# CPJKU/audio_sheet_retrieval

Measured on AMD Instinct MI355X. Metric: snippet-pairs/sec embedded+ranked (32-d CCA), higher is better.
Workload: dtype f32

## Files before the change

### audio_sheet_retrieval_amd/csrc/conv_wino4_kernels.hip

```cpp
#include <hip/hip_runtime.h>
#include <stdint.h>
#include <stdlib.h>
#include <algorithm>
#include <type_traits>
#include <vector>
#include "asr_kernels.h"
#include "repack_elems.inl"
#include "wino4_epilogue.h"

#ifndef ASR_WINO4_ABL
#define ASR_WINO4_ABL 0
#endif

namespace asr {

typedef float floatx4q __attribute__((ext_vector_type(4)));
typedef float float2q __attribute__((ext_vector_type(2)));

struct Wino4Args {
    const float *in, *wpk, *bnp;
    float *out;
    int N, H, W, OH, OW;
    int ty_img, tx_img;
    int coutp;
    int tiles;
    int total;
    double *stats;
    BnBwdFuse bf;
    int epi;
};

__device__ __forceinline__ float elu_fastq(float y) { return y > 0.0f ? y : __expf(y) - 1.0f; }

__device__ __forceinline__ floatx4q bn_elu4q(floatx4q x, float mean, float scale, float beta) {
    const floatx4q y = (x - floatx4q{mean, mean, mean, mean}) * floatx4q{scale, scale, scale, scale} +
                       floatx4q{beta, beta, beta, beta};
    return floatx4q{elu_fastq(y[0]), elu_fastq(y[1]), elu_fastq(y[2]), elu_fastq(y[3])};
}
typedef int int4q __attribute__((ext_vector_type(4)));
__device__ __forceinline__ void buffer_store_q(float v, unsigned voff, int4q rsrc, unsigned soff) {
    asm volatile("buffer_store_dword %0, %1, %2, %3 offen" ::"v"(v), "v"(voff), "s"(rsrc), "s"(soff) : "memory");
}

template <typename T> __device__ __forceinline__ T splatq(float c);
template <> __device__ __forceinline__ float2q splatq<float2q>(float c) { return float2q{c, c}; }
template <> __device__ __forceinline__ floatx4q splatq<floatx4q>(float c) { return floatx4q{c, c, c, c}; }
template <typename T> __device__ __forceinline__ T fmaq(float c, T x, T y) {
    return __builtin_elementwise_fma(splatq<T>(c), x, y);
}

template <typename T> __device__ __forceinline__ void in6(T &d0, T &d1, T &d2, T &d3, T &d4, T &d5) {
    const T r0 = fmaq(4.f, d0, fmaq(-5.f, d2, d4));
    const T t1 = fmaq(-4.f, d2, d4), t2 = fmaq(-4.f, d1, d3);
    const T t3 = d4 - d2, t4 = d3 - d1;
    const T r5 = fmaq(4.f, d1, fmaq(-5.f, d3, d5));
    d0 = r0; d1 = t1 + t2; d2 = t1 - t2; d3 = fmaq(2.f, t4, t3); d4 = fmaq(-2.f, t4, t3); d5 = r5;
}
template <typename T> __device__ __forceinline__ void out6(T m0, T m1, T m2, T m3, T m4, T m5, T &y0, T &y1, T &y2, T &y3) {
    const T s1 = m1 + m2, s2 = m1 - m2, s3 = m3 + m4, s4 = m3 - m4;
    y0 = (m0 + s1) + s3;
    y1 = fmaq(2.f, s4, s2);
    y2 = fmaq(4.f, s3, s1);
    y3 = fmaq(8.f, s4, s2) + m5;
}

template <int CIN, int COUT, bool POOL, int WAVES, bool RAW>
__global__ __launch_bounds__(64 * WAVES, 1) void conv3x3_wino4g(Wino4Args a) {
    constexpr int KS = CIN / 4, NB = CIN / 8, T = 64 * WAVES;
    constexpr int WS = 16;
    constexpr int WD = 6;
    constexpr int WQ = 72;
    static_assert(CIN % 8 == 0, "channel blocks of 8");
    extern __shared__ __align__(16) float w_lds[];
    const int tid = threadIdx.x, lane = tid & 63;
    const int wave = __builtin_amdgcn_readfirstlane(tid >> 6);
    const int nt0 = blockIdx.y;
    for (int i = tid; i < KS * 36 * 4 * 16; i += T) {
        const int row = i >> 4, nn = i & 15;
        const int gg = row & 3, kp = row >> 2, ks = kp / 36, p = kp - ks * 36;
        const int qq = (ks & 1) * 36 + p;
        w_lds[i] = a.wpk[((((size_t)(ks >> 1) * 18 + (qq >> 2)) * 4 + gg) * a.coutp + nt0 * 16 + nn) * 4 + (qq & 3)];
    }
    __syncthreads();

    const int m = lane & 15, g = lane >> 4, n = lane & 15;
    const float *w_lane = w_lds + g * WS + n;
    const int chn = nt0 * 16 + n;
    const bool ch_ok = chn < COUT;
    const float bmean = (!RAW && ch_ok) ? a.bnp[chn] : 0.f;
    const float bscale = (!RAW && ch_ok) ? a.bnp[a.coutp + chn] : 1.f;
    const float bbeta = (!RAW && ch_ok) ? a.bnp[2 * a.coutp + chn] : 0.f;
    const int per_img = a.ty_img * a.tx_img;

    for (int mt = blockIdx.x * WAVES + wave; mt < a.total; mt += gridDim.x * WAVES) {
        const int tnum = mt * 16 + m;
        const bool tvalid = tnum < a.tiles;
        const int tcl = min(tnum, a.tiles - 1);
        const int img = tcl / per_img;
        const int trest = tcl - img * per_img;
        const int tty = trest / a.tx_img, ttx = trest - tty * a.tx_img;
        const int py = 4 * tty, px = 4 * ttx;
        const float *ibase = a.in + (int64_t)img * a.H * a.W * CIN + 2 * g;
        int rowb[6], colb[6];
        unsigned oy_m = 0, ox_m = 0;
#pragma unroll
        for (int i = 0; i < 6; ++i) {
            const int y = py - 1 + i, x = px - 1 + i;
            oy_m |= (unsigned)(y >= 0 && y < a.H) << i;
            ox_m |= (unsigned)(x >= 0 && x < a.W) << i;
            rowb[i] = min(max(y, 0), a.H - 1) * a.W * CIN;
            colb[i] = min(max(x, 0), a.W - 1) * CIN;
        }
        if (!tvalid) oy_m = 0;
        const bool interior = __builtin_amdgcn_ballot_w64(oy_m != 0x3fu || ox_m != 0x3fu) == 0;
        unsigned my_off;
        int my_ext;
        if (POOL) {
            my_off = (((unsigned)img * a.OH + 2 * tty) * a.OW + 2 * ttx) * COUT;
            const int nr = min(2, a.OH - 2 * tty), nc = min(2, a.OW - 2 * ttx);
            my_ext = (tvalid && nr > 0 && nc > 0) ? (nr | (nc << 8)) : 0;
        } else {
            my_off = (((unsigned)img * a.H + py) * a.W + px) * COUT;
            const int nr = min(4, a.H - py), nc = min(4, a.W - px);
            my_ext = tvalid ? (nr | (nc << 8)) : 0;
        }

        floatx4q acc[36];
#pragma unroll
        for (int p = 0; p < 36; ++p) acc[p] = floatx4q{0.f, 0.f, 0.f, 0.f};

        float2q nxt[6][6];
#pragma unroll
        for (int i = 0; i < 6; ++i)
#pragma unroll
            for (int j = 0; j < 6; ++j) nxt[i][j] = *reinterpret_cast<const float2q *>(ibase + rowb[i] + colb[j]);
        float wpre[WD];
#pragma unroll
        for (int q = 0; q < WD; ++q) wpre[q] = w_lane[q * 4 * WS];
#pragma unroll 1
        for (int t = 0; t < NB; ++t) {
            float2q dp[6][6];
            if (interior) {
#pragma unroll
                for (int i = 0; i < 6; ++i)
#pragma unroll
                    for (int j = 0; j < 6; ++j) dp[i][j] = nxt[i][j];
            } else {
#pragma unroll
                for (int i = 0; i < 6; ++i)
#pragma unroll
                    for (int j = 0; j < 6; ++j)
                        dp[i][j] = (((oy_m >> i) & (ox_m >> j)) & 1u) ? nxt[i][j] : float2q{0.f, 0.f};
            }
            if (t + 1 < NB && !(ASR_WINO4_ABL & 2)) {
#pragma unroll
                for (int i = 0; i < 6; ++i)
#pragma unroll
                    for (int j = 0; j < 6; ++j)
                        nxt[i][j] = *reinterpret_cast<const float2q *>(ibase + rowb[i] + colb[j] + 8 * (t + 1));
            }
#pragma unroll
            for (int j = 0; j < 6; ++j) in6(dp[0][j], dp[1][j], dp[2][j], dp[3][j], dp[4][j], dp[5][j]);
#pragma unroll
            for (int i = 0; i < 6; ++i) in6(dp[i][0], dp[i][1], dp[i][2], dp[i][3], dp[i][4], dp[i][5]);
            const float *wk = w_lane + (2 * t) * (36 * 4 * WS);
            const float *wn = (t + 1 < NB) ? wk + 2 * 36 * 4 * WS : w_lane;
            float wv[WQ + WD];
#pragma unroll
            for (int q = 0; q < WD; ++q) wv[q] = wpre[q];
#pragma unroll
            for (int q0 = 0; q0 < WQ; q0 += 2) {
#pragma unroll
                for (int q = q0; q < q0 + 2; ++q)
                    wv[q + WD] = (q + WD < WQ) ? wk[(q + WD) * 4 * WS] : wn[(q + WD - WQ) * 4 * WS];
                __builtin_amdgcn_sched_barrier(0);
#pragma unroll
                for (int q = q0; q < q0 + 2; ++q) {
                    const int c = q / 36, p = q % 36;
                    acc[p] = __builtin_amdgcn_mfma_f32_16x16x4f32(dp[p / 6][p % 6][c], wv[q], acc[p], 0, 0, 0);
                }
                __builtin_amdgcn_sched_barrier(0);
            }
#pragma unroll
            for (int q = 0; q < WD; ++q) wpre[q] = wv[WQ + q];
        }

        unsigned eo[4];
        int ee[4];
#pragma unroll
        for (int r = 0; r < 4; ++r) {
            eo[r] = (unsigned)__shfl((int)my_off, 4 * g + r);
            ee[r] = __shfl(my_ext, 4 * g + r);
        }
        if (!ch_ok) continue;
        floatx4q tc[4][6];
#pragma unroll
        for (int nu = 0; nu < 6; ++nu)
            out6(acc[nu], acc[6 + nu], acc[12 + nu], acc[18 + nu], acc[24 + nu], acc[30 + nu], tc[0][nu], tc[1][nu], tc[2][nu],
                 tc[3][nu]);
        if (POOL) {
#pragma unroll
            for (int pr = 0; pr < 2; ++pr) {
                floatx4q ya[4], yb[4];
                out6(tc[2 * pr][0], tc[2 * pr][1], tc[2 * pr][2], tc[2 * pr][3], tc[2 * pr][4], tc[2 * pr][5], ya[0], ya[1],
                     ya[2], ya[3]);
                out6(tc[2 * pr + 1][0], tc[2 * pr + 1][1], tc[2 * pr + 1][2], tc[2 * pr + 1][3], tc[2 * pr + 1][4],
                     tc[2 * pr + 1][5], yb[0], yb[1], yb[2], yb[3]);
#pragma unroll
                for (int pc = 0; pc < 2; ++pc) {
#pragma unroll
                    for (int r = 0; r < 4; ++r) {
                        if (pr >= (ee[r] & 0xff) || pc >= (ee[r] >> 8)) continue;
                        const float v0 = ya[2 * pc][r], v1 = ya[2 * pc + 1][r], v2 = yb[2 * pc][r], v3 = yb[2 * pc + 1][r];
                        const float hi = fmaxf(fmaxf(v0, v1), fmaxf(v2, v3));
                        const float lo = fminf(fminf(v0, v1), fminf(v2, v3));
                        const float x = bscale >= 0.0f ? hi : lo;
                        a.out[(size_t)eo[r] + (size_t)(pr * a.OW + pc) * COUT + chn] =
                            elu_fastq((x - bmean) * bscale + bbeta);
                    }
                }
            }
        } else {
#pragma unroll
            for (int i = 0; i < 4; ++i) {
                floatx4q y[4];
                out6(tc[i][0], tc[i][1], tc[i][2], tc[i][3], tc[i][4], tc[i][5], y[0], y[1], y[2], y[3]);
#pragma unroll
                for (int j = 0; j < 4; ++j) {
#pragma unroll
                    for (int r = 0; r < 4; ++r) {
                        if (i >= (ee[r] & 0xff) || j >= (ee[r] >> 8)) continue;
                        const float v = RAW ? y[j][r] : elu_fastq((y[j][r] - bmean) * bscale + bbeta);
                        a.out[(size_t)eo[r] + (size_t)(i * a.W + j) * COUT + chn] = v;
                    }
                }
            }
        }
    }
}

template <int CIN, int COUT, bool POOL, int SLICE = COUT, int PW = 1, bool RAW = false>
__global__ __launch_bounds__(64 * (PW + (SLICE + 15) / 16), 1) void conv3x3_wino4s(Wino4Args a) {
    static_assert(!(RAW && POOL), "the raw form has no pooled epilogue");
    constexpr int NT = (SLICE + 15) / 16, NB = CIN / 8, KS = CIN / 4;
    static_assert(PW == 1 || PW == 2, "one or two producer waves");
    static_assert(PW + NT <= 4, "one wave per SIMD");
    static_assert(SLICE == COUT || (SLICE % 16 == 0 && COUT % SLICE == 0), "slices are whole n-tiles");
    constexpr int VB = 36 * 16 * 8;
    static_assert(CIN % 8 == 0, "channel blocks of 8");
    extern __shared__ __align__(16) float vbuf[];
    const int tid = threadIdx.x, lane = tid & 63;
    const int wave = __builtin_amdgcn_readfirstlane(tid >> 6);
    const bool producer = wave < PW;
    const int m = lane & 15, g = lane >> 4, n = lane & 15;
    const int per_img = a.ty_img * a.tx_img;

    int mt, mt_end, mt_stride;
    if ((gridDim.x & 7) == 0) {
        const int per_x = (a.total + 7) >> 3;
        const int r0 = (int)(blockIdx.x & 7) * per_x;
        mt_end = min(r0 + per_x, a.total);
        mt_stride = (int)(gridDim.x >> 3);
        mt = r0 + (int)(blockIdx.x >> 3);
    } else {
        mt_end = a.total; mt_stride = (int)gridDim.x; mt = (int)blockIdx.x;
    }
    if (mt >= mt_end) {
        if constexpr (RAW) {
            if (a.stats)
                for (int c = threadIdx.x; c < 2 * COUT; c += blockDim.x) a.stats[(size_t)blockIdx.x * 2 * COUT + c] = 0.0;
        }
        return;
    }

    auto tile_of = [&](int mtile, int &img, int &tty, int &ttx, bool &tvalid) {
        const int tnum = mtile * 16 + m;
        tvalid = tnum < a.tiles;
        const int tcl = min(tnum, a.tiles - 1);
        img = tcl / per_img;
        const int trest = tcl - img * per_img;
        tty = trest / a.tx_img;
        ttx = trest - tty * a.tx_img;
    };
    float *vlane = vbuf + (g * 32 + 2 * m);
#ifdef ASR_WINO4_OLD_V
    vlane = vbuf + (m * 8 + 2 * g);
#endif

    if (producer) {
        unsigned poff[6][6];
        unsigned oy_m = 0, ox_m = 0;
        auto setup = [&](int mtile) {
            int img, tty, ttx;
            bool tvalid;
            tile_of(mtile, img, tty, ttx, tvalid);
            const int py = 4 * tty, px = 4 * ttx;
            const unsigned ib = ((unsigned)img * a.H * a.W * CIN + 2 * g) * 4u;
            unsigned rowb[6], colb[6];
            oy_m = 0; ox_m = 0;
#pragma unroll
            for (int i = 0; i < 6; ++i) {
                const int y = py - 1 + i, x = px - 1 + i;
                oy_m |= (unsigned)(y >= 0 && y < a.H) << i;
                ox_m |= (unsigned)(x >= 0 && x < a.W) << i;
                rowb[i] = (unsigned)(min(max(y, 0), a.H - 1) * a.W * CIN) * 4u;
                colb[i] = (unsigned)(min(max(x, 0), a.W - 1) * CIN) * 4u;
            }
            if (!tvalid) oy_m = 0;
#pragma unroll
            for (int i = 0; i < 6; ++i)
#pragma unroll
                for (int j = 0; j < 6; ++j) poff[i][j] = ib + rowb[i] + colb[j];
        };
        float2q nxt[6][6];
        auto load = [&](int t) {
            const char *cb = reinterpret_cast<const char *>(a.in + 8 * t);
#pragma unroll
            for (int i = 0; i < 6; ++i)
#pragma unroll
                for (int j = 0; j < 6; ++j) nxt[i][j] = *reinterpret_cast<const float2q *>(cb + poff[i][j]);
        };
        const int n_mt = (mt_end - mt + mt_stride - 1) / mt_stride;
        const int n_steps = n_mt * NB;
        int passed = 0;
        int t = wave;
        while (t >= NB) { t -= NB; mt += mt_stride; }
        if (mt < mt_end) { setup(mt); load(t); }
        for (int step = wave; step < n_steps; step += PW) {
            float2q dp[6][6];
            const unsigned oy = oy_m, ox = ox_m;
            const bool interior = __builtin_amdgcn_ballot_w64(oy != 0x3fu || ox != 0x3fu) == 0;
            if (interior) {
#pragma unroll
                for (int i = 0; i < 6; ++i)
#pragma unroll
                    for (int j = 0; j < 6; ++j) dp[i][j] = nxt[i][j];
            } else {
#pragma unroll
                for (int i = 0; i < 6; ++i)
#pragma unroll
                    for (int j = 0; j < 6; ++j) dp[i][j] = (((oy >> i) & (ox >> j)) & 1u) ? nxt[i][j] : float2q{0.f, 0.f};
            }
            {
                int tn = t + PW, mtn = mt;
                while (tn >= NB) { tn -= NB; mtn += mt_stride; }
                if (!(ASR_WINO4_ABL & 2) && step + PW < n_steps) {
                    if (mtn != mt) setup(mtn);
                    load(tn);
                }
                t = tn; mt = mtn;
            }
            if (!(ASR_WINO4_ABL & 8)) {
#pragma unroll
            for (int j = 0; j < 6; ++j) in6(dp[0][j], dp[1][j], dp[2][j], dp[3][j], dp[4][j], dp[5][j]);
#pragma unroll
            for (int i = 0; i < 6; ++i) in6(dp[i][0], dp[i][1], dp[i][2], dp[i][3], dp[i][4], dp[i][5]);
            }
            while (passed < step) { __syncthreads(); ++passed; }
            float *vb = vlane + (step & 1) * VB;
            if (!(ASR_WINO4_ABL & 16)) {
#pragma unroll
            for (int p = 0; p < 36; ++p) *reinterpret_cast<float2q *>(vb + p * 128) = dp[p / 6][p % 6];
            } else {
#pragma unroll
            for (int p = 0; p < 36; ++p) asm volatile("" ::"v"(dp[p / 6][p % 6]));
            }
            __syncthreads();
            ++passed;
        }
        while (passed < n_steps + 1) { __syncthreads(); ++passed; }
        return;
    }

    const int nt = wave - PW;
    const int chn = (int)blockIdx.y * SLICE + nt * 16 + n;
    const bool ch_ok = chn < COUT;
    float bmean = (!RAW && ch_ok) ? a.bnp[chn] : 0.f;
    float bscale = (!RAW && ch_ok) ? a.bnp[a.coutp + chn] : 1.f;
    float bbeta = (!RAW && ch_ok) ? a.bnp[2 * a.coutp + chn] : 0.f;
    float bistd = 0.f;
    const bool bnb = ASR_BNB_FUSE_BUILD && RAW && a.stats && a.bf.z != nullptr;
    if (bnb && ch_ok) {
        bmean = a.bf.cst[chn]; bistd = a.bf.cst[COUT + chn];
        bscale = a.bf.cst[2 * COUT + chn]; bbeta = a.bf.cst[3 * COUT + chn];
    }
    double st1 = 0.0, st2 = 0.0;
    int4q orsrc;
    {
        const uint64_t obase = reinterpret_cast<uint64_t>(a.out);
        orsrc.x = (int)(uint32_t)obase;
        orsrc.y = (int)(uint32_t)(obase >> 32);
        orsrc.z = (int)((unsigned)a.N * a.OH * a.OW * COUT * 4u);
        orsrc.w = 0x00020000;
    }
    const unsigned wlane = ((unsigned)g * a.coutp + chn) * 16u;
    const float *wl = a.wpk;
    constexpr int wstep = 4 * ((COUT + 15) / 16 * 16);
    floatx4q bw[2][18];
#pragma unroll
    for (int j = 0; j < 18; ++j)
        bw[0][j] = *reinterpret_cast<const floatx4q *>(reinterpret_cast<const char *>(wl) + (size_t)j * (wstep * 16) + wlane);
    int step = 0;
    for (; mt < mt_end; mt += mt_stride) {
        unsigned my_off;
        int my_ext;
        {
            int img, tty, ttx;
            bool tvalid;
            tile_of(mt, img, tty, ttx, tvalid);
            if (POOL) my_off = (((unsigned)img * a.OH + 2 * tty) * a.OW + 2 * ttx) * COUT;
            else my_off = (((unsigned)img * a.H + 4 * tty) * a.W + 4 * ttx) * COUT;
            my_ext = wino4_extent(POOL, POOL ? a.OH : a.H, POOL ? a.OW : a.W, tty, ttx, tvalid);
        }
        int epi_mode = 0;
        if constexpr (!RAW) {
            if (a.epi)
                epi_mode = __builtin_amdgcn_ballot_w64(!wino4_rows_full(my_ext, POOL)) == 0 ? 1 : (wino4_general_form(POOL) ? 2 : 0);
        }
        unsigned voff[9];
#pragma unroll
        for (int k = 0; k < 9; ++k) {
            voff[k] = wlane + (unsigned)k * (2 * wstep * 16);
            asm volatile("" : "+v"(voff[k]));
        }
        floatx4q acc[36];
        auto reload = [&](const float *wn, auto set_c) {
            constexpr int SET = decltype(set_c)::value;
            if (ASR_WINO4_ABL & 4) return;
            const char *wnb = reinterpret_cast<const char *>(wn);
#pragma unroll
            for (int k = 0; k < 9; ++k) {
                unsigned vo = voff[k];
                asm volatile("" : "+v"(vo));
                bw[SET][2 * k] = *reinterpret_cast<const floatx4q *>(wnb + vo);
                bw[SET][2 * k + 1] = *reinterpret_cast<const floatx4q *>(wnb + (wstep * 16) + vo);
            }
        };
        auto run_step = [&](const float *vb, const float *wn, auto cur_c, auto first) {
            constexpr bool FIRST = decltype(first)::value;
            constexpr int CUR = decltype(cur_c)::value;
            using NXT = std::integral_constant<int, CUR ^ 1>;
            __syncthreads();
            reload(wn, NXT{});
            __builtin_amdgcn_sched_barrier(0);
            float2q dp[2][12];
#pragma unroll
            for (int i = 0; i < 12; ++i) dp[0][i] = *reinterpret_cast<const float2q *>(vb + i * 128);
#pragma unroll
            for (int grp = 0; grp < 3; ++grp) {
                if (grp < 2) {
#pragma unroll
                    for (int i = 0; i < 12; ++i)
                        dp[(grp + 1) & 1][i] = *reinterpret_cast<const float2q *>(vb + ((grp + 1) * 12 + i) * 128);
                }
#pragma unroll
                for (int c = 0; c < 2; ++c)
#pragma unroll
                    for (int i = 0; i < 12; ++i) {
                        const int p = grp * 12 + i;
                        if (FIRST && c == 0)
                            acc[p] = __builtin_amdgcn_mfma_f32_16x16x4f32(dp[grp & 1][i][c], bw[CUR][(c * 36 + p) >> 2][(c * 36 + p) & 3],
                                                                          floatx4q{0.f, 0.f, 0.f, 0.f}, 0, 0, 0);
                        else
                            acc[p] = __builtin_amdgcn_mfma_f32_16x16x4f32(dp[grp & 1][i][c], bw[CUR][(c * 36 + p) >> 2][(c * 36 + p) & 3], acc[p],
                                                                          0, 0,
                                                                          0);
                    }
                __builtin_amdgcn_sched_barrier(0);
            }
        };
        using C0 = std::integral_constant<int, 0>;
        using C1 = std::integral_constant<int, 1>;
        auto wblock = [&](int t) {
            unsigned blk = (unsigned)(((t + 1) % NB) * 72) * wstep;
            asm volatile("" : "+s"(blk));
            return wl + blk;
        };
        run_step(vlane + (step & 1) * VB, wblock(0), C0{}, std::true_type{});
        ++step;
#pragma unroll 1
        for (int t = 1; t + 1 < NB; t += 2) {
            run_step(vlane + (step & 1) * VB, wblock(t), C1{}, std::false_type{});
            ++step;
            run_step(vlane + (step & 1) * VB, wblock(t + 1), C0{}, std::false_type{});
            ++step;
        }
        if constexpr ((NB & 1) == 0) {
            run_step(vlane + (step & 1) * VB, wblock(NB - 1), C1{}, std::false_type{});
            ++step;
        } else {
#pragma unroll
            for (int j = 0; j < 18; ++j) bw[0][j] = bw[1][j];
        }

        unsigned eo[4];
        int ee[4];
#pragma unroll
        for (int r = 0; r < 4; ++r) {
            eo[r] = (unsigned)__shfl((int)my_off, 4 * g + r);
            ee[r] = __shfl(my_ext, 4 * g + r);
        }
        if (!ch_ok) continue;
        floatx4q tc[4][6];
#pragma unroll
        for (int nu = 0; nu < 6; ++nu)
            out6(acc[nu], acc[6 + nu], acc[12 + nu], acc[18 + nu], acc[24 + nu], acc[30 + nu], tc[0][nu], tc[1][nu], tc[2][nu],
                 tc[3][nu]);
        auto fast_epilogue = [&](auto rows_c) {
            constexpr bool ROWS = decltype(rows_c)::value;
            constexpr int SP = POOL ? 2 : 4;
            unsigned vo[4][SP];
#pragma unroll
            for (int r = 0; r < 4; ++r)
#pragma unroll
                for (int c = 0; c < SP; ++c) vo[r][c] = wino4_store_offset(eo[r], ee[r], chn, c, COUT);
#pragma unroll
            for (int i = 0; i < SP; ++i) {
                const unsigned soff = wino4_row_bytes(i, a.OW, COUT);
                floatx4q res[SP];
                if constexpr (POOL) {
                    floatx4q ya[4], yb[4];
                    out6(tc[2 * i][0], tc[2 * i][1], tc[2 * i][2], tc[2 * i][3], tc[2 * i][4], tc[2 * i][5], ya[0], ya[1], ya[2],
                         ya[3]);
                    out6(tc[2 * i + 1][0], tc[2 * i + 1][1], tc[2 * i + 1][2], tc[2 * i + 1][3], tc[2 * i + 1][4],
                         tc[2 * i + 1][5], yb[0], yb[1], yb[2], yb[3]);
#pragma unroll
                    for (int pc = 0; pc < 2; ++pc) {
                        const floatx4q hi = __builtin_elementwise_max(__builtin_elementwise_max(ya[2 * pc], ya[2 * pc + 1]),
                                                                      __builtin_elementwise_max(yb[2 * pc], yb[2 * pc + 1]));
                        const floatx4q lo = __builtin_elementwise_min(__builtin_elementwise_min(ya[2 * pc], ya[2 * pc + 1]),
                                                                      __builtin_elementwise_min(yb[2 * pc], yb[2 * pc + 1]));
                        res[pc] = bn_elu4q(bscale >= 0.0f ? hi : lo, bmean, bscale, bbeta);
                    }
                } else {
                    floatx4q y[4];
                    out6(tc[i][0], tc[i][1], tc[i][2], tc[i][3], tc[i][4], tc[i][5], y[0], y[1], y[2], y[3]);
#pragma unroll
                    for (int j = 0; j < 4; ++j) res[j] = bn_elu4q(y[j], bmean, bscale, bbeta);
                }
#pragma unroll
                for (int j = 0; j < SP; ++j)
#pragma unroll
                    for (int r = 0; r < 4; ++r) {
                        if (ASR_WINO4_ABL & 32) asm volatile("" ::"v"(res[j][r]));
                        else buffer_store_q(res[j][r], ROWS ? wino4_store_offset_row(vo[r][j], ee[r], i) : vo[r][j], orsrc, soff);
                    }
            }
        };
        if (epi_mode == 1) { fast_epilogue(std::false_type{}); continue; }
        if constexpr (!RAW && wino4_general_form(POOL)) {
            if (epi_mode == 2) { fast_epilogue(std::true_type{}); continue; }
        }
        if (POOL) {
#pragma unroll
            for (int pr = 0; pr < 2; ++pr) {
                floatx4q ya[4], yb[4];
                out6(tc[2 * pr][0], tc[2 * pr][1], tc[2 * pr][2], tc[2 * pr][3], tc[2 * pr][4], tc[2 * pr][5], ya[0], ya[1],
                     ya[2], ya[3]);
                out6(tc[2 * pr + 1][0], tc[2 * pr + 1][1], tc[2 * pr + 1][2], tc[2 * pr + 1][3], tc[2 * pr + 1][4],
                     tc[2 * pr + 1][5], yb[0], yb[1], yb[2], yb[3]);
#pragma unroll
                for (int pc = 0; pc < 2; ++pc) {
#pragma unroll
                    for (int r = 0; r < 4; ++r) {
                        if (pr >= (ee[r] & 0xff) || pc >= (ee[r] >> 8)) continue;
                        const float v0 = ya[2 * pc][r], v1 = ya[2 * pc + 1][r], v2 = yb[2 * pc][r], v3 = yb[2 * pc + 1][r];
                        const float hi = fmaxf(fmaxf(v0, v1), fmaxf(v2, v3));
                        const float lo = fminf(fminf(v0, v1), fminf(v2, v3));
                        const float x = bscale >= 0.0f ? hi : lo;
                        const float res = elu_fastq((x - bmean) * bscale + bbeta);
                        if (ASR_WINO4_ABL & 32) asm volatile("" ::"v"(res));
                        else a.out[(size_t)eo[r] + (size_t)(pr * a.OW + pc) * COUT + chn] = res;
                    }
                }
            }
        } else {
#pragma unroll
            for (int i = 0; i < 4; ++i) {
                floatx4q y[4];
                out6(tc[i][0], tc[i][1], tc[i][2], tc[i][3], tc[i][4], tc[i][5], y[0], y[1], y[2], y[3]);
                float rs1 = 0.f, rs2 = 0.f;
#pragma unroll
                for (int j = 0; j < 4; ++j) {
#pragma unroll
                    for (int r = 0; r < 4; ++r) {
                        if (i >= (ee[r] & 0xff) || j >= (ee[r] >> 8)) continue;
                        const float res = RAW ? y[j][r] : elu_fastq((y[j][r] - bmean) * bscale + bbeta);
                        if (RAW) {
                            if (bnb) {
                                const size_t e = (size_t)eo[r] + (size_t)(i * a.W + j) * COUT + chn;
                                bnb_acc(res, a.bf.z[e], bnb_mult(a.bf.tie, e), bmean, bscale, bbeta, bistd, rs1, rs2);
                            } else { rs1 += res; rs2 = fmaf(res, res, rs2); }
                        }
                        if (ASR_WINO4_ABL & 32) asm volatile("" ::"v"(res));
                        else a.out[(size_t)eo[r] + (size_t)(i * a.W + j) * COUT + chn] = res;
                    }
                }
                if (RAW) { st1 += (double)rs1; st2 += (double)rs2; }
            }
        }
    }
    __syncthreads();
    if constexpr (RAW) {
        if (a.stats) {
            st1 += __shfl_xor(st1, 16); st2 += __shfl_xor(st2, 16);
            st1 += __shfl_xor(st1, 32); st2 += __shfl_xor(st2, 32);
            if (g == 0 && ch_ok) {
                a.stats[((size_t)blockIdx.x * 2) * COUT + chn] = st1;
                a.stats[((size_t)blockIdx.x * 2 + 1) * COUT + chn] = st2;
            }
        }
    }
}

__global__ void wino4_pack_kernel(const float *W, int cin, int cout, int dgrad, float *wpk) {
    const int idx = blockIdx.x * blockDim.x + threadIdx.x;
    if (idx >= wino4_pack_count(cin, cout, dgrad)) return;
    wino4_pack_elem(idx, W, cin, cout, dgrad, wpk);
}

size_t wino4_wpack_floats(int cin, int cout) { return (cin % 8) ? 0 : (size_t)36 * cin * ((cout + 15) / 16 * 16); }

hipError_t launch_wino4_pack(hipStream_t s, const float *W, int cin, int cout, float *wpk, int dgrad) {
    const int kdim = dgrad ? cout : cin, ndim = dgrad ? cin : cout;
    if (kdim % 8) return hipSuccess;
    const int total = kdim * ((ndim + 15) / 16 * 16);
    hipLaunchKernelGGL(wino4_pack_kernel, dim3((total + 255) / 256), dim3(256), 0, s, W, cin, cout, dgrad, wpk);
    return hipGetLastError();
}

struct Wino4Variant {
    int cin, cout, pool, waves, raw;
    void (*kernel)(Wino4Args);
    const char *symbol;
    int spec;
    int slice;
};
#define ASR_BOOLSTRQ_0 "false"
#define ASR_BOOLSTRQ_1 "true"
#define ASR_WINO4(CIN, COUT, POOL, WAVES)                                                                         \
    { CIN, COUT, POOL, WAVES, 0, conv3x3_wino4g<CIN, COUT, (POOL != 0), WAVES, false>,                            \
      "void asr::conv3x3_wino4g<" #CIN ", " #COUT ", " ASR_BOOLSTRQ_##POOL ", " #WAVES ", false>(asr::Wino4Args)" }
#define ASR_WINO4S(CIN, COUT, POOL)                                                                               \
    { CIN, COUT, POOL, 1 + (COUT + 15) / 16, 0, conv3x3_wino4s<CIN, COUT, (POOL != 0)>,                           \
      "void asr::conv3x3_wino4s<" #CIN ", " #COUT ", " ASR_BOOLSTRQ_##POOL ", " #COUT ", 1, false>(asr::Wino4Args)", 1, 0 }
#define ASR_WINO4S2(CIN, COUT, POOL)                                                                              \
    { CIN, COUT, POOL, 2 + (COUT + 15) / 16, 0, conv3x3_wino4s<CIN, COUT, (POOL != 0), COUT, 2>,                  \
      "void asr::conv3x3_wino4s<" #CIN ", " #COUT ", " ASR_BOOLSTRQ_##POOL ", " #COUT ", 2, false>(asr::Wino4Args)", 1, 0 }
#define ASR_WINO4SR(CIN, COUT)                                                                                    \
    { CIN, COUT, 0, 1 + (COUT + 15) / 16, 1, conv3x3_wino4s<CIN, COUT, false, COUT, 1, true>,                     \
      "void asr::conv3x3_wino4s<" #CIN ", " #COUT ", false, " #COUT ", 1, true>(asr::Wino4Args)", 1, 0 }
#define ASR_WINO4SL(CIN, COUT, POOL, SLICE)                                                                       \
    { CIN, COUT, POOL, 1 + SLICE / 16, 0, conv3x3_wino4s<CIN, COUT, (POOL != 0), SLICE>,                          \
      "void asr::conv3x3_wino4s<" #CIN ", " #COUT ", " ASR_BOOLSTRQ_##POOL ", " #SLICE ", 1, false>(asr::Wino4Args)", 1, SLICE }
static const Wino4Variant g_wino4[] = {
    ASR_WINO4(24, 24, 1, 4), ASR_WINO4(24, 48, 0, 4), ASR_WINO4(48, 48, 1, 4), ASR_WINO4(48, 48, 0, 4),
    ASR_WINO4S(24, 24, 1), ASR_WINO4S(24, 48, 0), ASR_WINO4S(48, 48, 1), ASR_WINO4S(48, 48, 0),
    ASR_WINO4S2(24, 24, 1),
    ASR_WINO4SL(48, 96, 0, 48), ASR_WINO4SL(96, 96, 1, 48), ASR_WINO4SL(96, 96, 0, 48),
    ASR_WINO4SR(24, 48), ASR_WINO4SR(48, 48), ASR_WINO4SR(48, 24),
};
static const int g_num_wino4 = (int)(sizeof(g_wino4) / sizeof(g_wino4[0]));

void conv_candidates_wino4(int cin, int cout, int pool, int H, int W, std::vector<ConvPlan> *out) {
    static const int use = getenv("ASR_CONV_WINO4") ? atoi(getenv("ASR_CONV_WINO4")) : -1;
    if (use == 0) return;
    const int epi = getenv("ASR_WINO4_EPI") ? (atoi(getenv("ASR_WINO4_EPI")) != 0) : 1;
    for (int vi = 0; vi < g_num_wino4; ++vi) {
        const Wino4Variant &v = g_wino4[vi];
        if (v.cin != cin || v.cout != cout || v.pool != pool || v.raw) continue;
        if (!v.spec && use != 1) continue;
        const int lds = v.spec ? 2 * 36 * 16 * 8 * 4 : 36 * cin * 16 * 4;
        (void)hipFuncSetAttribute(reinterpret_cast<const void *>(v.kernel), hipFuncAttributeMaxDynamicSharedMemorySize,
                                  160 * 1024);
        int nb = 0;
        if (hipOccupancyMaxActiveBlocksPerMultiprocessor(&nb, reinterpret_cast<const void *>(v.kernel), 64 * v.waves,
                                                         (size_t)lds) != hipSuccess || nb < 1) {
            (void)hipGetLastError();
            nb = 1;
        }
        ConvPlan bp{};
        bp.cin = cin; bp.cout = cout; bp.pool = pool;
        bp.H = H; bp.W = W; bp.OH = pool ? H / 2 : H; bp.OW = pool ? W / 2 : W;
        bp.TH = 4; bp.TW = 64; bp.NI = 16;
        bp.tiles_y = ((pool ? 2 * bp.OH : H) + 3) / 4; bp.tiles_x = ((pool ? 2 * bp.OW : W) + 3) / 4;
        bp.threads = 64 * v.waves;
        bp.lds_bytes = lds;
        bp.blocks_per_cu = v.spec ? 1 : std::min(nb, 4);
        bp.cost = (double)bp.tiles_y * bp.tiles_x / 16.0 * ((cout + 15) / 16) * (36.0 * (cin / 4) * 32.0 + 3000.0) *
                  (v.spec ? 0.4 : 1.0);
        bp.variant = 4000 + vi;
        bp.symbol = v.symbol;
        bp.epi = v.spec ? epi : 0;
        out->push_back(bp);
    }
}

void conv_candidates_wino4_raw(int cin, int cout, int H, int W, std::vector<ConvPlan> *out, int dgrad) {
    static const int use = getenv("ASR_TRAIN_WINO4") ? atoi(getenv("ASR_TRAIN_WINO4")) : -1;
    if (use == 0 || (use == 5 && !dgrad)) return;
    for (int vi = 0; vi < g_num_wino4; ++vi) {
        const Wino4Variant &v = g_wino4[vi];
        if (v.cin != cin || v.cout != cout || !v.raw) continue;
        const int lds = 2 * 36 * 16 * 8 * 4;
        (void)hipFuncSetAttribute(reinterpret_cast<const void *>(v.kernel), hipFuncAttributeMaxDynamicSharedMemorySize,
                                  160 * 1024);
        ConvPlan bp{};
        bp.cin = cin; bp.cout = cout; bp.pool = 0;
        bp.H = H; bp.W = W; bp.OH = H; bp.OW = W;
        bp.TH = 4; bp.TW = 64; bp.NI = 16;
        bp.tiles_y = (H + 3) / 4; bp.tiles_x = (W + 3) / 4;
        bp.threads = 64 * v.waves;
        bp.lds_bytes = lds;
        bp.blocks_per_cu = 1;
        bp.cost = (double)bp.tiles_y * bp.tiles_x / 16.0 * ((cout + 15) / 16) * (36.0 * (cin / 4) * 32.0 + 3000.0) * 0.4;
        bp.variant = 4000 + vi;
        bp.symbol = v.symbol;
        out->push_back(bp);
    }
}
bool conv_wino4_is_raw(const ConvPlan &p) { return p.variant >= 4000 && g_wino4[p.variant - 4000].raw != 0; }
int conv_wino4_stats_rows_max(int num_cus) { return num_cus; }

hipError_t launch_conv_wino4(hipStream_t s, const ConvPlan &p, const float *in, const float *wpk, const float *bnp,
                             float *out, int N, int num_cus, double *stats, int *stats_rows, bool stats_clean,
                             const BnBwdFuse *bf) {
    const Wino4Variant &v = g_wino4[p.variant - 4000];
    Wino4Args a;
    a.epi = (p.epi && v.spec && !v.raw && wino4_fast_epilogue_admitted(N, p.OH, p.OW, p.cout)) ? 1 : 0;
    a.stats = nullptr;
    a.bf = BnBwdFuse{nullptr, nullptr, nullptr};
    a.in = in; a.wpk = wpk; a.bnp = bnp; a.out = out;
    a.N = N; a.H = p.H; a.W = p.W; a.OH = p.OH; a.OW = p.OW;
    a.ty_img = p.tiles_y; a.tx_img = p.tiles_x;
    a.coutp = (p.cout + 15) / 16 * 16;
    a.tiles = N * a.ty_img * a.tx_img;
    a.total = (a.tiles + 15) / 16;
    if (a.total == 0) return hipSuccess;
    if (v.spec) {
        if ((double)N * p.H * p.W * p.cin * 4.0 >= 4294967296.0) return hipErrorInvalidValue;
        const int slices = v.slice ? p.cout / v.slice : 1;
        int grid = std::min(a.total, std::max(1, num_cus * std::max(1, p.blocks_per_cu) / slices));
        if (grid >= 8) grid &= ~7;
        if (v.raw && stats) {
            a.stats = stats;
            if (bf) a.bf = *bf;
            (void)stats_clean;
            if (stats_rows) *stats_rows = grid;
        }
        hipLaunchKernelGGL(v.kernel, dim3(grid, slices), dim3(p.threads), p.lds_bytes, s, a);
        return hipGetLastError();
    }
    const int ntiles = a.coutp / 16;
    const int waves = p.threads / 64;
    const int slots = std::max(1, num_cus * std::max(1, p.blocks_per_cu) / ntiles);
    const int grid = std::min((a.total + waves - 1) / waves, slots);
    hipLaunchKernelGGL(v.kernel, dim3(grid, ntiles), dim3(p.threads), p.lds_bytes, s, a);
    return hipGetLastError();
}

}
```

Measured before the change: 314,300.

## Group two channel blocks per barrier step in specialized Winograd-4 conv

Producer and consumer waves in the warp-specialized Winograd F(4,3) kernel now exchange two 8-channel blocks per barrier step instead of one, for single-producer variants with an even block count. The LDS ring grows from 2 to 4 slots and the consumer skips every other __syncthreads, halving block-wide barriers per M-tile. The aim is to cut barrier stalls between producer and consumers, at the cost of doubled LDS use and a longer producer lead that may add latency.

Result: no change. 316,200, median of 6 (+0.6%).

```diff
diff --git a/audio_sheet_retrieval_amd/csrc/conv_wino4_kernels.hip b/audio_sheet_retrieval_amd/csrc/conv_wino4_kernels.hip
--- a/audio_sheet_retrieval_amd/csrc/conv_wino4_kernels.hip
+++ b/audio_sheet_retrieval_amd/csrc/conv_wino4_kernels.hip
@@ -7,6 +7,7 @@
 #include "asr_kernels.h"
 #include "repack_elems.inl"
 #include "wino4_epilogue.h"
+#include "wino4_step_layout.h"
 
 #ifndef ASR_WINO4_ABL
 #define ASR_WINO4_ABL 0
@@ -246,7 +247,8 @@
     static_assert(PW == 1 || PW == 2, "one or two producer waves");
     static_assert(PW + NT <= 4, "one wave per SIMD");
     static_assert(SLICE == COUT || (SLICE % 16 == 0 && COUT % SLICE == 0), "slices are whole n-tiles");
-    constexpr int VB = 36 * 16 * 8;
+    constexpr int SW = wino4_step_width(CIN, PW);
+    static_assert(NB % SW == 0, "a step stays inside its M-tile");
     static_assert(CIN % 8 == 0, "channel blocks of 8");
     extern __shared__ __align__(16) float vbuf[];
     const int tid = threadIdx.x, lane = tid & 63;
@@ -321,12 +323,12 @@
                 for (int j = 0; j < 6; ++j) nxt[i][j] = *reinterpret_cast<const float2q *>(cb + poff[i][j]);
         };
         const int n_mt = (mt_end - mt + mt_stride - 1) / mt_stride;
-        const int n_steps = n_mt * NB;
+        const int n_items = n_mt * NB;
         int passed = 0;
         int t = wave;
         while (t >= NB) { t -= NB; mt += mt_stride; }
         if (mt < mt_end) { setup(mt); load(t); }
-        for (int step = wave; step < n_steps; step += PW) {
+        for (int item = wave; item < n_items; item += PW) {
             float2q dp[6][6];
             const unsigned oy = oy_m, ox = ox_m;
             const bool interior = __builtin_amdgcn_ballot_w64(oy != 0x3fu || ox != 0x3fu) == 0;
@@ -344,7 +346,7 @@
             {
                 int tn = t + PW, mtn = mt;
                 while (tn >= NB) { tn -= NB; mtn += mt_stride; }
-                if (!(ASR_WINO4_ABL & 2) && step + PW < n_steps) {
+                if (!(ASR_WINO4_ABL & 2) && item + PW < n_items) {
                     if (mtn != mt) setup(mtn);
                     load(tn);
                 }
@@ -356,8 +358,9 @@
 #pragma unroll
             for (int i = 0; i < 6; ++i) in6(dp[i][0], dp[i][1], dp[i][2], dp[i][3], dp[i][4], dp[i][5]);
             }
+            const int step = wino4_item_step(SW, item);
             while (passed < step) { __syncthreads(); ++passed; }
-            float *vb = vlane + (step & 1) * VB;
+            float *vb = vlane + wino4_item_offset(SW, item);
             if (!(ASR_WINO4_ABL & 16)) {
 #pragma unroll
             for (int p = 0; p < 36; ++p) *reinterpret_cast<float2q *>(vb + p * 128) = dp[p / 6][p % 6];
@@ -365,10 +368,12 @@
 #pragma unroll
             for (int p = 0; p < 36; ++p) asm volatile("" ::"v"(dp[p / 6][p % 6]));
             }
-            __syncthreads();
-            ++passed;
-        }
-        while (passed < n_steps + 1) { __syncthreads(); ++passed; }
+            if (wino4_item_closes_step(SW, item)) {
+                __syncthreads();
+                ++passed;
+            }
+        }
+        while (passed < wino4_barriers(SW, n_items)) { __syncthreads(); ++passed; }
         return;
     }
 
@@ -400,7 +405,7 @@
 #pragma unroll
     for (int j = 0; j < 18; ++j)
         bw[0][j] = *reinterpret_cast<const floatx4q *>(reinterpret_cast<const char *>(wl) + (size_t)j * (wstep * 16) + wlane);
-    int step = 0;
+    int item = 0;
     for (; mt < mt_end; mt += mt_stride) {
         unsigned my_off;
         int my_ext;
@@ -440,7 +445,7 @@
             constexpr bool FIRST = decltype(first)::value;
             constexpr int CUR = decltype(cur_c)::value;
             using NXT = std::integral_constant<int, CUR ^ 1>;
-            __syncthreads();
+            if constexpr (SW == 1 || CUR == 0) __syncthreads();
             reload(wn, NXT{});
             __builtin_amdgcn_sched_barrier(0);
             float2q dp[2][12];
@@ -476,18 +481,18 @@
             asm volatile("" : "+s"(blk));
             return wl + blk;
         };
-        run_step(vlane + (step & 1) * VB, wblock(0), C0{}, std::true_type{});
-        ++step;
+        run_step(vlane + wino4_item_offset(SW, item), wblock(0), C0{}, std::true_type{});
+        ++item;
 #pragma unroll 1
         for (int t = 1; t + 1 < NB; t += 2) {
-            run_step(vlane + (step & 1) * VB, wblock(t), C1{}, std::false_type{});
-            ++step;
-            run_step(vlane + (step & 1) * VB, wblock(t + 1), C0{}, std::false_type{});
-            ++step;
+            run_step(vlane + wino4_item_offset(SW, item), wblock(t), C1{}, std::false_type{});
+            ++item;
+            run_step(vlane + wino4_item_offset(SW, item), wblock(t + 1), C0{}, std::false_type{});
+            ++item;
         }
         if constexpr ((NB & 1) == 0) {
-            run_step(vlane + (step & 1) * VB, wblock(NB - 1), C1{}, std::false_type{});
-            ++step;
+            run_step(vlane + wino4_item_offset(SW, item), wblock(NB - 1), C1{}, std::false_type{});
+            ++item;
         } else {
 #pragma unroll
             for (int j = 0; j < 18; ++j) bw[0][j] = bw[1][j];
@@ -635,7 +640,11 @@
     const char *symbol;
     int spec;
     int slice;
+    int pw;
 };
+static int wino4_lds_bytes(const Wino4Variant &v) {
+    return v.spec ? wino4_v_lds_bytes(wino4_step_width(v.cin, v.pw)) : 36 * v.cin * 16 * 4;
+}
 #define ASR_BOOLSTRQ_0 "false"
 #define ASR_BOOLSTRQ_1 "true"
 #define ASR_WINO4(CIN, COUT, POOL, WAVES)                                                                         \
@@ -643,16 +652,16 @@
       "void asr::conv3x3_wino4g<" #CIN ", " #COUT ", " ASR_BOOLSTRQ_##POOL ", " #WAVES ", false>(asr::Wino4Args)" }
 #define ASR_WINO4S(CIN, COUT, POOL)                                                                               \
     { CIN, COUT, POOL, 1 + (COUT + 15) / 16, 0, conv3x3_wino4s<CIN, COUT, (POOL != 0)>,                           \
-      "void asr::conv3x3_wino4s<" #CIN ", " #COUT ", " ASR_BOOLSTRQ_##POOL ", " #COUT ", 1, false>(asr::Wino4Args)", 1, 0 }
+      "void asr::conv3x3_wino4s<" #CIN ", " #COUT ", " ASR_BOOLSTRQ_##POOL ", " #COUT ", 1, false>(asr::Wino4Args)", 1, 0, 1 }
 #define ASR_WINO4S2(CIN, COUT, POOL)                                                                              \
     { CIN, COUT, POOL, 2 + (COUT + 15) / 16, 0, conv3x3_wino4s<CIN, COUT, (POOL != 0), COUT, 2>,                  \
-      "void asr::conv3x3_wino4s<" #CIN ", " #COUT ", " ASR_BOOLSTRQ_##POOL ", " #COUT ", 2, false>(asr::Wino4Args)", 1, 0 }
+      "void asr::conv3x3_wino4s<" #CIN ", " #COUT ", " ASR_BOOLSTRQ_##POOL ", " #COUT ", 2, false>(asr::Wino4Args)", 1, 0, 2 }
 #define ASR_WINO4SR(CIN, COUT)                                                                                    \
     { CIN, COUT, 0, 1 + (COUT + 15) / 16, 1, conv3x3_wino4s<CIN, COUT, false, COUT, 1, true>,                     \
-      "void asr::conv3x3_wino4s<" #CIN ", " #COUT ", false, " #COUT ", 1, true>(asr::Wino4Args)", 1, 0 }
+      "void asr::conv3x3_wino4s<" #CIN ", " #COUT ", false, " #COUT ", 1, true>(asr::Wino4Args)", 1, 0, 1 }
 #define ASR_WINO4SL(CIN, COUT, POOL, SLICE)                                                                       \
     { CIN, COUT, POOL, 1 + SLICE / 16, 0, conv3x3_wino4s<CIN, COUT, (POOL != 0), SLICE>,                          \
-      "void asr::conv3x3_wino4s<" #CIN ", " #COUT ", " ASR_BOOLSTRQ_##POOL ", " #SLICE ", 1, false>(asr::Wino4Args)", 1, SLICE }
+      "void asr::conv3x3_wino4s<" #CIN ", " #COUT ", " ASR_BOOLSTRQ_##POOL ", " #SLICE ", 1, false>(asr::Wino4Args)", 1, SLICE, 1 }
 static const Wino4Variant g_wino4[] = {
     ASR_WINO4(24, 24, 1, 4), ASR_WINO4(24, 48, 0, 4), ASR_WINO4(48, 48, 1, 4), ASR_WINO4(48, 48, 0, 4),
     ASR_WINO4S(24, 24, 1), ASR_WINO4S(24, 48, 0), ASR_WINO4S(48, 48, 1), ASR_WINO4S(48, 48, 0),
@@ -670,7 +679,7 @@
         const Wino4Variant &v = g_wino4[vi];
         if (v.cin != cin || v.cout != cout || v.pool != pool || v.raw) continue;
         if (!v.spec && use != 1) continue;
-        const int lds = v.spec ? 2 * 36 * 16 * 8 * 4 : 36 * cin * 16 * 4;
+        const int lds = wino4_lds_bytes(v);
         (void)hipFuncSetAttribute(reinterpret_cast<const void *>(v.kernel), hipFuncAttributeMaxDynamicSharedMemorySize,
                                   160 * 1024);
         int nb = 0;
@@ -702,7 +711,7 @@
     for (int vi = 0; vi < g_num_wino4; ++vi) {
         const Wino4Variant &v = g_wino4[vi];
         if (v.cin != cin || v.cout != cout || !v.raw) continue;
-        const int lds = 2 * 36 * 16 * 8 * 4;
+        const int lds = wino4_lds_bytes(v);
         (void)hipFuncSetAttribute(reinterpret_cast<const void *>(v.kernel), hipFuncAttributeMaxDynamicSharedMemorySize,
                                   160 * 1024);
         ConvPlan bp{};
@@ -748,7 +757,7 @@
             (void)stats_clean;
             if (stats_rows) *stats_rows = grid;
         }
-        hipLaunchKernelGGL(v.kernel, dim3(grid, slices), dim3(p.threads), p.lds_bytes, s, a);
+        hipLaunchKernelGGL(v.kernel, dim3(grid, slices), dim3(p.threads), wino4_lds_bytes(v), s, a);
         return hipGetLastError();
     }
     const int ntiles = a.coutp / 16;
diff --git a/audio_sheet_retrieval_amd/csrc/wino4_step_layout.h b/audio_sheet_retrieval_amd/csrc/wino4_step_layout.h
--- /dev/null
+++ b/audio_sheet_retrieval_amd/csrc/wino4_step_layout.h
@@ -0,0 +1,34 @@
+#pragma once
+
+#if defined(__HIPCC__)
+#define ASR_W4STEP_HD __host__ __device__ __forceinline__ constexpr
+#else
+#define ASR_W4STEP_HD inline constexpr
+#endif
+
+#ifndef ASR_WINO4_STEP16
+#define ASR_WINO4_STEP16 1
+#endif
+
+namespace asr {
+
+ASR_W4STEP_HD int wino4_v_floats() { return 36 * 16 * 8; }
+
+ASR_W4STEP_HD int wino4_step_width(int cin, int pw) {
+    return (ASR_WINO4_STEP16 && pw == 1 && (cin / 8) % 2 == 0) ? 2 : 1;
+}
+
+ASR_W4STEP_HD int wino4_v_slots(int width) { return 2 * width; }
+ASR_W4STEP_HD int wino4_v_lds_bytes(int width) { return wino4_v_slots(width) * wino4_v_floats() * 4; }
+
+ASR_W4STEP_HD int wino4_item_step(int width, int item) { return (int)((unsigned)item / (unsigned)width); }
+ASR_W4STEP_HD int wino4_item_offset(int width, int item) {
+    return (int)((unsigned)item % (unsigned)wino4_v_slots(width)) * wino4_v_floats();
+}
+ASR_W4STEP_HD bool wino4_item_closes_step(int width, int item) {
+    return (unsigned)item % (unsigned)width == (unsigned)width - 1u;
+}
+
+ASR_W4STEP_HD int wino4_barriers(int width, int n_items) { return n_items / width + 1; }
+
+}
```
